# AITRICS/Medical_Tri_Modal_Pilot

Measured on AMD Instinct MI355X. Metric: tri-modal training samples/s (fwd+bwd+AdamW step, per-GPU batch 64), higher is better.
Workload: dtype bf16; 1 GPU; BASELINE configs[1]: vslt_img_txt tri_mbt_vsltcls, 6 layers, d_model 256, batch 64/GPU, TIE-len 1000 (N_v=1005), 224x224 CXR, 128-tok text, dropout 0.1, mbt-only-vslt 1, imgtxt-time 1; global_batch=64, parallelism=dp1

## Files before the change

### include/mtmp.h

```cpp
#ifndef MTMP_H
#define MTMP_H
#include <stdint.h>
#ifdef __cplusplus
extern "C" {
#endif

#define MTMP_F32 0
#define MTMP_BF16 1

int mtmp_abi_version(void);
const char* mtmp_last_error(void);

int mtmp_attn_fwd(int dtype, const void* q, const void* k, const void* v, void* o, const void* res, void* o_res,
                  float* lse, const int32_t* kv_len, const float* key_norms, int B, int N, int H, int ld_qkv, int ld_o,
                  float scale, void* stream);
int mtmp_attn_fwd_grouped(int dtype, int n, const void* const* q, const void* const* k, const void* const* v, void* const* o,
                          const void* const* res, void* const* o_res, float* const* lse, const int32_t* const* kv_len,
                          const int32_t* const* row_start, const float* const* key_norms, const int* N, const int* ld_qkv,
                          const int* ld_o, int B, int H, float scale, void* stream);
int mtmp_attn_bwd_grouped(int dtype, int n, const void* const* q, const void* const* k, const void* const* v,
                          const void* const* o, const void* const* d_o, const float* const* lse, const int32_t* const* kv_len,
                          const int32_t* const* row_start, void* const* dq, void* const* dk, void* const* dv,
                          float* const* delta_ws, const int* N, const int* ld_qkv, const int* ld_o, const int* ld_do,
                          const int* ld_dqkv, int B, int H, float scale, void* stream);
int mtmp_attn_cls_fwd(int dtype, const void* q, const void* k, const void* v, int ld_qkv, const void* res, int ld_res, void* o_cls,
                      void* r1_cls, float* lse, const int32_t* kv_len, const int32_t* row_start, int B, int N, int H, int cls_tok,
                      float scale, void* stream);
int mtmp_attn_cls_bwd(int dtype, const void* q, const void* k, const void* v, int ld_qkv, const void* o_cls, const void* d_o,
                      const float* lse, const int32_t* kv_len, const int32_t* row_start, void* dq, void* dk, void* dv, int ld_dqkv,
                      int B, int N, int H, int cls_tok, float scale, void* stream);
long long mtmp_key_norms_floats(long long rows, int H);
int mtmp_key_norms(int dtype, const void* k, float* out, long long rows, int H, int ld, void* stream);

int mtmp_attn_bwd(int dtype, const void* q, const void* k, const void* v, const void* o, const void* d_o,
                  const float* lse, const int32_t* kv_len, void* dq, void* dk, void* dv, float* delta_ws, int B,
                  int N, int H, int ld_qkv, int ld_o, int ld_do, int ld_dqkv, float scale, void* stream);

int mtmp_ln_gemm(int dtype, const void* x, const float* gamma, const float* beta, const void* w, const float* bias,
                 void* y, void* xn, float* stats, int M, int N, int ldx, int ldy, float eps, int relu, float drop_p,
                 unsigned seed, const unsigned* seed_dev, void* stream);

int mtmp_ln_gemm_qkv(int dtype, const void* x, const float* gamma, const float* beta, const void* w, const float* bias,
                     void* y, void* xn, float* stats, float* key_norms, int M, int ldx, float eps, void* stream);

int mtmp_gemm_nt(int dtype, const void* a, const void* w, const float* bias, const void* res, void* y, int M, int N,
                 int K, int lda, int ldy, int ldr, int act, float drop_p, unsigned seed, const unsigned* seed_dev,
                 const void* gate, float gate_scale, const float* row_scale, int rows_per_scale, void* stream);

long long mtmp_sign_bits_bytes(int M, int N);
int mtmp_ln_gemm_signs(int dtype, const void* x, const float* gamma, const float* beta, const void* w, const float* bias,
                       void* y, void* xn, float* stats, int M, int N, int ldx, int ldy, float eps, float drop_p,
                       unsigned seed, const unsigned* seed_dev, void* signs, void* stream);
int mtmp_gemm_nt_signs(int dtype, const void* a, const void* w, void* y, int M, int N, int lda, int ldy,
                       const void* signs, float gate_scale, void* stream);
int mtmp_gemm_nt_signs_drop(int dtype, const void* a, const void* w, void* y, int M, int N, int lda, int ldy,
                            const void* signs, float gate_scale, float drop_p, unsigned seed, const unsigned* seed_dev,
                            void* a_out, void* stream);

long long mtmp_gemm_tn_ws_floats(int M, int N, int K);
int mtmp_gemm_tn(int dtype, const void* dy, const void* x, float* dw, float* db, float* ws, int M, int N, int K,
                 int ldy, int ldx, void* stream);
int mtmp_gemm_tn_live(int dtype, const void* dy, const void* x, float* dw, float* db, float* ws, int M, int N, int K,
                      int ldy, int ldx, const int32_t* rows_live, void* stream);

int mtmp_dropout_bwd(int dtype, const void* g_in, void* g_out, long long n, unsigned seed, const unsigned* seed_dev,
                     float p, void* stream);

int mtmp_ln_bwd_ws_floats(int M);
int mtmp_ln_bwd(int dtype, const void* z, int ldz, const float* stats, const float* gamma, const void* dy,
                const void* d_res, int ldr, void* dz, float* dgamma_dbeta, float* ws, int M, float eps, void* stream);

int mtmp_gemm_lnbwd_ws_floats(int M);
int mtmp_gemm_lnbwd(int dtype, const void* dy, const void* wt, const void* z, int ldz, const float* stats,
                    const float* gamma, const void* d_res, int ldr, void* dz, float* dgamma_dbeta, float* ws, int M,
                    int K, int ldy, float eps, void* stream);

int mtmp_tie_embed_fwd(int dtype, const float* events, const float* params, const float* ftab, void* out, int n,
                       void* stream);
int mtmp_tie_bwd_ws_floats(int n);
int mtmp_tie_embed_bwd(int dtype, const float* events, const float* params, const void* d_out, float* grads,
                       float* ws, int n, void* stream);

int mtmp_time_embed_fwd(int dtype, const float* events, const float* params, const float* ftab, void* out, int n,
// ... 163 lines not shown
```

### medical_tri_modal_pilot_amd/_lib.py

```python
import ctypes
import os
from ctypes import c_char_p, c_float, c_int, c_longlong, c_uint, c_void_p

_HERE = os.path.dirname(os.path.abspath(__file__))
LIB_PATH = os.environ.get("MTMP_LIB", os.path.join(_HERE, "libmtmp_hip.so"))

F32, BF16 = 0, 1

SIGNATURES = {
    "mtmp_abi_version": (c_int, []),
    "mtmp_last_error": (c_char_p, []),
    "mtmp_attn_fwd": (c_int, [c_int] + [c_void_p] * 9 + [c_int] * 5 + [c_float, c_void_p]),
    "mtmp_attn_cls_fwd": (c_int, [c_int] + [c_void_p] * 3 + [c_int, c_void_p, c_int] + [c_void_p] * 5 + [c_int] * 4 + [c_float, c_void_p]),
    "mtmp_attn_cls_bwd": (c_int, [c_int] + [c_void_p] * 3 + [c_int] + [c_void_p] * 8 + [c_int] * 5 + [c_float, c_void_p]),
    "mtmp_attn_fwd_grouped": (c_int, [c_int, c_int] + [c_void_p] * 13 + [c_int, c_int, c_float, c_void_p]),
    "mtmp_attn_bwd_grouped": (c_int, [c_int, c_int] + [c_void_p] * 17 + [c_int, c_int, c_float, c_void_p]),
    "mtmp_key_norms_floats": (c_longlong, [c_longlong, c_int]),
    "mtmp_key_norms": (c_int, [c_int, c_void_p, c_void_p, c_longlong, c_int, c_int, c_void_p]),
    "mtmp_attn_bwd": (c_int, [c_int] + [c_void_p] * 11 + [c_int] * 7 + [c_float, c_void_p]),
    "mtmp_ln_gemm": (c_int, [c_int] + [c_void_p] * 8 + [c_int] * 4 + [c_float, c_int, c_float, c_uint, c_void_p, c_void_p]),
    "mtmp_ln_gemm_qkv": (c_int, [c_int] + [c_void_p] * 9 + [c_int, c_int, c_float, c_void_p]),
    "mtmp_gemm_nt": (c_int, [c_int] + [c_void_p] * 5 + [c_int] * 7 + [c_float, c_uint, c_void_p, c_void_p, c_float, c_void_p, c_int,
                             c_void_p]),
    "mtmp_gemm_nt_live": (c_int, [c_int] + [c_void_p] * 5 + [c_int] * 7 + [c_float, c_uint, c_void_p, c_void_p, c_float, c_void_p, c_int,
                             c_void_p, c_void_p]),
    "mtmp_sign_bits_bytes": (c_longlong, [c_int, c_int]),
    "mtmp_ln_gemm_signs": (c_int, [c_int] + [c_void_p] * 8 + [c_int] * 4 + [c_float, c_float, c_uint, c_void_p, c_void_p, c_void_p]),
    "mtmp_gemm_nt_signs": (c_int, [c_int] + [c_void_p] * 3 + [c_int] * 4 + [c_void_p, c_float, c_void_p]),
    "mtmp_gemm_nt_signs_drop": (c_int, [c_int] + [c_void_p] * 3 + [c_int] * 4 + [c_void_p, c_float, c_float, c_uint, c_void_p,
                                                                                   c_void_p, c_void_p]),
    "mtmp_ln_gemm_qkv_grouped": (c_int, [c_int, c_int] + [c_void_p] * 11 + [c_float, c_void_p, c_void_p]),
    "mtmp_ln_gemm_signs_grouped": (c_int, [c_int, c_int] + [c_void_p] * 10 + [c_int, c_void_p, c_float, c_float, c_void_p, c_void_p,
                                                                                   c_void_p, c_void_p]),
    "mtmp_gemm_nt_grouped": (c_int, [c_int, c_int] + [c_void_p] * 6 + [c_int, c_int] + [c_void_p] * 3 + [c_int, c_float, c_void_p,
                                                                                                       c_void_p, c_void_p, c_void_p]),
    "mtmp_gemm_nt_signs_drop_grouped": (c_int, [c_int, c_int] + [c_void_p] * 4 + [c_int, c_void_p, c_void_p, c_float, c_float,
                                                                                  c_void_p, c_void_p, c_void_p, c_void_p, c_void_p]),
    "mtmp_gemm_lnbwd_grouped": (c_int, [c_int, c_int] + [c_void_p] * 11 + [c_int, c_void_p, c_float, c_void_p, c_void_p]),
    "mtmp_gemm_tn_group_plan": (c_int, [c_int, c_void_p, c_int, c_int, c_void_p]),
    "mtmp_gemm_tn_grouped": (c_int, [c_int, c_int] + [c_void_p] * 4 + [c_int, c_int] + [c_void_p] * 4 + [c_void_p]),
    "mtmp_gemm_tn_slab_rows": (c_int, [c_int] * 4),
    "mtmp_gemm_lnbwd_slab_rows": (c_int, [c_int]),
    "mtmp_reduce_batch": (c_int, [c_void_p] * 6 + [c_int, c_void_p]),
    "mtmp_reduce_scatter": (c_int, [c_void_p] * 5 + [c_int, c_void_p]),
    "mtmp_stream_input_slab_rows": (c_int, [c_int]),
    "mtmp_stream_input_bwd_partials": (c_int, [c_int] + [c_void_p] * 7 + [c_int] * 3 + [c_float, c_uint, c_void_p, c_void_p, c_void_p, c_void_p]),
    "mtmp_stream_input_bwd_grouped": (c_int, [c_int, c_int] + [c_void_p] * 18),
    "mtmp_stream_input_fwd_add": (c_int, [c_int] + [c_void_p] * 8 + [c_int] * 3 + [c_float, c_float, c_uint, c_void_p, c_void_p, c_void_p, c_void_p, c_int, c_void_p]),
    "mtmp_token_sums": (c_int, [c_int, c_int] + [c_void_p] * 5),
    "mtmp_tie_bwd_slab_rows": (c_int, [c_int]),
    "mtmp_tie_time_embed_bwd_partials": (c_int, [c_int, c_void_p, c_int, c_void_p, c_int, c_int] + [c_void_p] * 6),
    "mtmp_publish_scalar": (c_int, [c_void_p, c_void_p, c_void_p]),
    "mtmp_copy_batch": (c_int, [c_void_p] * 4 + [c_int, c_void_p]),
    "mtmp_stream_lengths": (c_int, [c_void_p] * 4 + [c_int] * 3 + [c_void_p]),
    "mtmp_row_starts": (c_int, [c_void_p, c_void_p, c_int, c_int, c_void_p]),
    "mtmp_image_slots": (c_int, [c_void_p, c_int, c_void_p, c_int, c_int, c_void_p]),
    "mtmp_transpose_batch": (c_int, [c_int, c_void_p, c_void_p, c_void_p, c_void_p, c_int, c_void_p]),
    "mtmp_layernorm_rows": (c_int, [c_int] + [c_void_p] * 4 + [c_longlong, c_int, c_float, c_int, c_int, c_int, c_void_p]),
    "mtmp_layernorm_rows_live": (c_int, [c_int] + [c_void_p] * 4 + [c_longlong, c_int, c_float, c_int, c_int, c_int, c_void_p, c_void_p]),
    "mtmp_swin_window_attn": (c_int, [c_int] + [c_void_p] * 3 + [c_int] * 6 + [c_float, c_void_p]),
    "mtmp_swin_window_attn_live": (c_int, [c_int] + [c_void_p] * 3 + [c_int] * 6 + [c_float, c_void_p, c_void_p]),
    "mtmp_layernorm_rows_bwd_slab_rows": (c_int, [c_longlong, c_int]),
    "mtmp_layernorm_rows_bwd": (c_int, [c_int] + [c_void_p] * 5 + [c_longlong, c_int, c_float, c_void_p]),
    "mtmp_gelu_fwd": (c_int, [c_int, c_void_p, c_void_p, c_longlong, c_void_p]),
    "mtmp_gelu_bwd": (c_int, [c_int, c_void_p, c_void_p, c_void_p, c_longlong, c_void_p]),
    "mtmp_swin_window_attn_bwd": (c_int, [c_int] + [c_void_p] * 5 + [c_int] * 6 + [c_float, c_void_p]),
    "mtmp_swin_window_attn_pad": (c_int, [c_int] + [c_void_p] * 4 + [c_int] * 6 + [c_float, c_void_p, c_void_p]),
# ... 67 lines not shown
```

### medical_tri_modal_pilot_amd/ops.py

```python
import contextlib
import ctypes
from typing import Optional

import torch

from . import _lib, tuning
from ._lib import BF16, F32, call

LN_EPS = 1e-6
N_HEAD, D_MODEL, D_HEAD = 4, 256, 64


def _dt(t: torch.Tensor) -> int:
    if t.dtype == torch.float32:
        return F32
    if t.dtype == torch.bfloat16:
        return BF16
    raise TypeError(f"libmtmp_hip kernels take float32 or bfloat16, got {t.dtype}")


def _p(t: Optional[torch.Tensor], byte_offset: int = 0):
    return None if t is None else ctypes.c_void_p(t.data_ptr() + byte_offset)


# ... 1208 lines not shown
        dqkv = attn_bwd(qkv, o, dr1.view(B, N, D), lse, kv_len).view(M, 3 * D)
    else:
        dqkv = attn_bwd_grouped([qkv], [o], [_packed_full(dr1, B, N)], [lse], [kv_len], [pack])[0].view(M, 3 * D)[:live]
    dwqkv, dbqkv = gemm_tn(dqkv, xn1, out=(sink.wqkv, sink.bqkv) if direct else None, defer=red)
    dz, dg1, db1 = gemm_lnbwd(dqkv, wqkvt, z.view(M, D)[:live], st1, g1, d_res2d=dr1, gb_out=sink.gb1 if direct else None, defer=red)
    if late is not None and red:
        late.append((red, sink if direct else None))
    else:
        if red:
            reduce_batch(red)
        if direct:
            sink.flat.mark_ready(sink.idx)
    dz = dz.view(B, N, D) if pack is None else _packed_full(dz, B, N)
    if direct:
        return dz, None
    grads = (dg1, db1, dwqkv[:D], dbqkv[:D], dwqkv[D:2 * D], dbqkv[D:2 * D], dwqkv[2 * D:], dbqkv[2 * D:],
             dg2, db2, dw1, dc1, dw2, dc2)
    return dz, grads


def attn_cls_fwd(qkv, z, kv_len, pack, cls_tok):
    _gpu(qkv, z)
    B, N, _ = qkv.shape
    es = qkv.element_size()
    o = torch.empty(B, D_MODEL, dtype=qkv.dtype, device=qkv.device)
    r1 = torch.empty_like(o)
    lse = torch.empty(B, N_HEAD, dtype=torch.float32, device=qkv.device)
    call("mtmp_attn_cls_fwd", _dt(qkv), _p(qkv), _p(qkv, D_MODEL * es), _p(qkv, 2 * D_MODEL * es), qkv.stride(1), _p(z), z.stride(1),
         _p(o), _p(r1), _p(lse), _p(kv_len), _p(pack), B, N, N_HEAD, int(cls_tok), D_HEAD ** -0.5, _stream())
    return o, r1, lse


def attn_cls_bwd(qkv, o_cls, d_o, lse, kv_len, pack, cls_tok):
    _gpu(qkv, o_cls, d_o)
    B, N, _ = qkv.shape
    es = qkv.element_size()
    dqkv = torch.empty_like(qkv)
    call("mtmp_attn_cls_bwd", _dt(qkv), _p(qkv), _p(qkv, D_MODEL * es), _p(qkv, 2 * D_MODEL * es), qkv.stride(1), _p(o_cls), _p(_c(d_o)),
         _p(lse), _p(kv_len), _p(pack), _p(dqkv), _p(dqkv, D_MODEL * es), _p(dqkv, 2 * D_MODEL * es), dqkv.stride(1), B, N, N_HEAD,
         int(cls_tok), D_HEAD ** -0.5, _stream())
    return dqkv


_cls_rows_cache = {}


def _cls_rows(B, N, cls_tok, dev):
    key = (B, N, cls_tok, dev.type, dev.index)
    if key not in _cls_rows_cache:
        _cls_rows_cache[key] = (torch.arange(B, dtype=torch.int64) * N + cls_tok).to(dev)
    return _cls_rows_cache[key]


def cls_layer_forward(z, kv_len, P, fused, drop_p, seeds, pack, cls_tok):
    B, N, D = z.shape
    g1, b1, g2, b2, c1, c2 = P[0], P[1], P[8], P[9], P[11], P[13]
    wqkv, bqkv, w1c, w2c, w2t, wqkvt, w1t = fused
    z2 = z.view(B * N, D)
    if pack is not None:
        qkv, xn1, st1 = (t[0] for t in ln_gemm_qkv_grouped([z2], [g1], [b1], [wqkv], [bqkv], [pack])[:3])
    else:
        qkv, xn1, st1 = ln_gemm(z2, g1, b1, wqkv, bqkv, 3 * D)
    qkv = qkv.view(B, N, 3 * D)
    o_cls, r1, lse = attn_cls_fwd(qkv, z, kv_len, pack, cls_tok)
    h, xn2, st2, hsign = ln_gemm(r1, g2, b2, w1c, c1, 4 * D, relu=True, drop_p=drop_p, seed=seeds[0], want_signs=True)
    out = gemm_nt(h, w2c, c2, res2d=r1, drop_p=drop_p, seed=seeds[1])
    rows = pack[:B] if pack is not None else _cls_rows(B, N, cls_tok, z.device)
    return out, (z, kv_len, g1, g2, wqkvt, w1t, w2t, xn1, st1, qkv, o_cls, lse, r1, xn2, st2, h, drop_p, seeds, hsign, pack, rows, cls_tok)


def cls_layer_backward(saved, d_cls, sink=None, late=None):
    z, kv_len, g1, g2, wqkvt, w1t, w2t, xn1, st1, qkv, o_cls, lse, r1, xn2, st2, h, p, seeds, hsign, pack, rows, cls_tok = saved
    B, N, D = z.shape
    M = B * N
    d_out = _c(d_cls).to(z.dtype)
    direct = sink is not None and sink.usable()
    red = [] if tuning.DEFER_REDUCTIONS else None
    if hsign is not None and p > 0 and tuning.FOLD_DROPOUT_BWD:
        dh, dy2 = gemm_nt_signs(d_out, w2t, hsign, 1.0 / (1.0 - p), drop_p=p, seed=seeds[1])
    else:
        dy2 = dropout_bwd(d_out, seeds[1], p) if p > 0 else d_out
        dh = gemm_nt_signs(dy2, w2t, hsign, 1.0 / (1.0 - p)) if hsign is not None else gemm_nt(dy2, w2t, gate=h, gate_scale=1.0 / (1.0 - p))
    dw2, dc2 = gemm_tn(dy2, h, out=(sink.w2, sink.c2) if direct else None, defer=red)
    dw1, dc1 = gemm_tn(dh, xn2, out=(sink.w1, sink.c1) if direct else None, defer=red)
    dr1, dg2, db2 = gemm_lnbwd(dh, w1t, r1, st2, g2, d_res2d=d_out, gb_out=sink.gb2 if direct else None, defer=red)
    dqkv = attn_cls_bwd(qkv, o_cls, dr1, lse, kv_len, pack, cls_tok).view(M, 3 * D)
    z2 = z.view(M, D)
    if pack is not None:
        dwqkv, dbqkv = gemm_tn_grouped([dqkv], [xn1], [(sink.wqkv, sink.bqkv) if direct else None], [red], [pack])[0]
        dz, dg1, db1 = gemm_lnbwd_grouped([dqkv], [wqkvt], [z2], [st1], [g1], [None], [sink.gb1 if direct else None], [red], [pack])[0]
    else:
        dwqkv, dbqkv = gemm_tn(dqkv, xn1, out=(sink.wqkv, sink.bqkv) if direct else None, defer=red)
        dz, dg1, db1 = gemm_lnbwd(dqkv, wqkvt, z2, st1, g1, d_res2d=None, gb_out=sink.gb1 if direct else None, defer=red)
    (dz[cls_tok:] if pack is not None else dz).index_add_(0, rows, dr1)
    if late is not None and red:
        late.append((red, sink if direct else None))
    else:
        if red:
            reduce_batch(red)
        if direct:
            sink.flat.mark_ready(sink.idx)
    if direct:
        return dz.view(B, N, D), None
    grads = (dg1, db1, dwqkv[:D], dbqkv[:D], dwqkv[D:2 * D], dbqkv[D:2 * D], dwqkv[2 * D:], dbqkv[2 * D:],
             dg2, db2, dw1, dc1, dw2, dc2)
    return dz.view(B, N, D), grads




def grouped_ok(z) -> bool:
    return tuning.GROUPED_LAUNCHES and z.dtype == torch.bfloat16


def layer_forward_grouped(zs, kv_lens, Ps, fuseds, drop_p, seeds, packs=None, ffn_rows=None):
    n = len(zs)
    B, D = zs[0].shape[0], D_MODEL
    Ns = [z.shape[1] for z in zs]
    packs = [None] * n if packs is None else list(packs)
    z2 = [z.view(B * N, D) for z, N in zip(zs, Ns)]
    qkv, xn1, st1, knorm = ln_gemm_qkv_grouped(z2, [P[0] for P in Ps], [P[1] for P in Ps], [f[0] for f in fuseds], [f[1] for f in fuseds],
                                               packs)
    qkv = [q.view(B, N, 3 * D) for q, N in zip(qkv, Ns)]
    o, r1, lse = attn_fwd_grouped(qkv, kv_lens, list(zs), knorm, packs)
# ... 363 lines not shown
```

Measured before the change: 8385 samples/s.

## Collapse CLS-only attention layer algebraically to avoid full QKV projection over all tokens

Adds a dedicated CLS-layer path. Only the CLS query is needed, so the query is folded through the key weights and LN gamma/beta, and scores come directly from layer-normed tokens. The value projection is applied once to the attention-weighted normalized input rather than to every row. This removes the full per-token LN+QKV GEMM and the materialized qkv tensor in both forward and backward, replacing them with chunked streaming kernels that do online softmax and partial reductions. It adds several small per-sample kernels and fp32 workspace, and changes accumulation order relative to the GEMM path.

```diff
diff --git a/include/mtmp.h b/include/mtmp.h
--- a/include/mtmp.h
+++ b/include/mtmp.h
@@ -29,6 +29,14 @@
 int mtmp_attn_cls_bwd(int dtype, const void* q, const void* k, const void* v, int ld_qkv, const void* o_cls, const void* d_o,
                       const float* lse, const int32_t* kv_len, const int32_t* row_start, void* dq, void* dk, void* dv, int ld_dqkv,
                       int B, int N, int H, int cls_tok, float scale, void* stream);
+int mtmp_cls_layer_chunk(void);
+long long mtmp_cls_layer_ws_floats(long long B, long long N);
+int mtmp_cls_layer_fwd(int dtype, const void* z, int ldz, const float* gamma, const float* beta, const void* wqkv,
+                       const void* wqkvt, const float* bqkv, const int32_t* kv_len, const int32_t* row_start, int B, int N,
+                       int cls_tok, float eps, float scale, float* ws, void* r1, void* stream);
+int mtmp_cls_layer_bwd(int dtype, const void* z, int ldz, const float* gamma, const float* beta, const void* wqkv,
+                       const void* wqkvt, const int32_t* kv_len, const int32_t* row_start, int B, int N, int cls_tok, float eps,
+                       float scale, float* ws, const void* d_o, void* dz, float* dwqkv, float* dbqkv, float* dgb, void* stream);
 long long mtmp_key_norms_floats(long long rows, int H);
 int mtmp_key_norms(int dtype, const void* k, float* out, long long rows, int H, int ld, void* stream);
 
diff --git a/medical_tri_modal_pilot_amd/_lib.py b/medical_tri_modal_pilot_amd/_lib.py
--- a/medical_tri_modal_pilot_amd/_lib.py
+++ b/medical_tri_modal_pilot_amd/_lib.py
@@ -13,6 +13,10 @@
     "mtmp_attn_fwd": (c_int, [c_int] + [c_void_p] * 9 + [c_int] * 5 + [c_float, c_void_p]),
     "mtmp_attn_cls_fwd": (c_int, [c_int] + [c_void_p] * 3 + [c_int, c_void_p, c_int] + [c_void_p] * 5 + [c_int] * 4 + [c_float, c_void_p]),
     "mtmp_attn_cls_bwd": (c_int, [c_int] + [c_void_p] * 3 + [c_int] + [c_void_p] * 8 + [c_int] * 5 + [c_float, c_void_p]),
+    "mtmp_cls_layer_chunk": (c_int, []),
+    "mtmp_cls_layer_ws_floats": (c_longlong, [c_longlong, c_longlong]),
+    "mtmp_cls_layer_fwd": (c_int, [c_int, c_void_p, c_int] + [c_void_p] * 7 + [c_int] * 3 + [c_float, c_float] + [c_void_p] * 3),
+    "mtmp_cls_layer_bwd": (c_int, [c_int, c_void_p, c_int] + [c_void_p] * 6 + [c_int] * 3 + [c_float, c_float] + [c_void_p] * 7),
     "mtmp_attn_fwd_grouped": (c_int, [c_int, c_int] + [c_void_p] * 13 + [c_int, c_int, c_float, c_void_p]),
     "mtmp_attn_bwd_grouped": (c_int, [c_int, c_int] + [c_void_p] * 17 + [c_int, c_int, c_float, c_void_p]),
     "mtmp_key_norms_floats": (c_longlong, [c_longlong, c_int]),
diff --git a/medical_tri_modal_pilot_amd/csrc/cls_layer.hip b/medical_tri_modal_pilot_amd/csrc/cls_layer.hip
--- /dev/null
+++ b/medical_tri_modal_pilot_amd/csrc/cls_layer.hip
@@ -0,0 +1,562 @@
+#include "common.hip.h"
+
+namespace {
+
+constexpr int D = 256, H = 4, DHD = 64;
+constexpr int CHUNK = 64;
+constexpr int GPB = 8;
+constexpr float LOG2E = 1.4426950408889634f;
+constexpr float NEG = -1e30f;
+
+template <typename T> struct ClsArgs {
+    const T* z; int ldz;
+    const float* gamma; const float* beta;
+    const T* wqkv; const T* wqkvt; const float* bqkv;
+    const int* kv_len; const int* row_start;
+    int B, N, cls_tok, nch;
+    float eps, scale;
+    float *xc, *q, *qt, *qg, *sc0, *P, *mvec, *lse, *stats, *scores, *part, *pml, *dm, *dmg, *dd, *dqt, *dq, *gb;
+    T* r1;
+    const T* d_o;
+    T* dz;
+    float *dwqkv, *dbqkv, *dgb;
+};
+
+struct Geo { bool none, uniform; int kvl, nrows; size_t row0; };
+template <typename T> MTMP_DEV Geo geo(const ClsArgs<T>& p, int b) {
+    Geo g;
+    const int kv_raw = p.kv_len ? p.kv_len[b] : p.N;
+    g.none = p.row_start && kv_raw <= p.cls_tok;
+    g.uniform = !g.none && kv_raw <= 0;
+    g.kvl = g.uniform ? p.N : min(kv_raw, p.N);
+    g.nrows = p.row_start ? max(min(kv_raw, p.N), 0) : p.N;
+    g.row0 = p.row_start ? (size_t)p.row_start[b] : (size_t)b * p.N;
+    return g;
+}
+
+template <typename T> MTMP_DEV void ld8(const T* ptr, float (&o)[8]) {
+    const Frag<T> f = frag_load<T>(ptr);
+#pragma unroll
+    for (int j = 0; j < 8; ++j) o[j] = to_f32(f.v[j]);
+}
+template <typename T> MTMP_DEV void st8(T* ptr, const float (&v)[8]) {
+    Frag<T> f;
+#pragma unroll
+    for (int j = 0; j < 8; ++j) f.v[j] = from_f32<T>(v[j]);
+    frag_store<T>(ptr, f);
+}
+MTMP_DEV void ld8w(const float* ptr, float (&o)[8]) {
+    const f32x4 a = ld4f(ptr), b = ld4f(ptr + 4);
+    o[0] = a[0]; o[1] = a[1]; o[2] = a[2]; o[3] = a[3]; o[4] = b[0]; o[5] = b[1]; o[6] = b[2]; o[7] = b[3];
+}
+MTMP_DEV float grp_sum(float v) {
+    v += dpp_row<0x128>(v);
+    v += dpp_row<0x124>(v);
+    v += dpp_row<0x122>(v);
+    v += dpp_row<0x121>(v);
+    const auto r = __builtin_amdgcn_permlane16_swap(__float_as_uint(v), __float_as_uint(v), false, false);
+    return __uint_as_float(r[0]) + __uint_as_float(r[1]);
+}
+MTMP_DEV float block_sum(float v, float* red) {
+    v = wave_sum(v);
+    __syncthreads();
+    if ((threadIdx.x & 63) == 0) red[threadIdx.x >> 6] = v;
+    __syncthreads();
+    return (red[0] + red[1]) + (red[2] + red[3]);
+}
+
+template <typename T> __global__ __launch_bounds__(256) void cls_prepare_kernel(ClsArgs<T> p) {
+    __shared__ float sx[D], sq[D], red[4];
+    const int b = blockIdx.x, t = threadIdx.x;
+    const Geo g = geo(p, b);
+    if (g.none) {
+        p.xc[b * D + t] = 0.f;
+        p.q[b * D + t] = 0.f;
+        for (int h = 0; h < H; ++h) { p.qt[(b * H + h) * D + t] = 0.f; p.qg[(b * H + h) * D + t] = 0.f; }
+        if (t < H) p.sc0[b * H + t] = 0.f;
+        return;
+    }
+    const float zc = to_f32(p.z[(g.row0 + p.cls_tok) * p.ldz + t]);
+    const float mean = block_sum(zc, red) * (1.0f / D);
+    const float d = zc - mean;
+    const float sigma = sqrtf(block_sum(d * d, red) * (1.0f / (D - 1)));
+    const float rs = 1.0f / (sigma + p.eps);
+    const float gm = p.gamma[t], be = p.beta[t];
+    const float x = fmaf(gm, d * rs, be);
+    sx[t] = x;
+    p.xc[b * D + t] = x;
+    __syncthreads();
+    float a = p.bqkv[t];
+#pragma unroll 8
+    for (int k = 0; k < D; ++k) a = fmaf(to_f32(p.wqkvt[(size_t)k * 3 * D + t]), sx[k], a);
+    sq[t] = a;
+    p.q[b * D + t] = a;
+    __syncthreads();
+    const float c2 = p.scale * LOG2E;
+    for (int h = 0; h < H; ++h) {
+        float w = 0.f;
+#pragma unroll 8
+        for (int dd = 0; dd < DHD; ++dd) w = fmaf(to_f32(p.wqkv[(size_t)(D + DHD * h + dd) * D + t]), sq[DHD * h + dd], w);
+        if (g.uniform) w = 0.f;
+        p.qt[(b * H + h) * D + t] = w;
+        p.qg[(b * H + h) * D + t] = w * c2 * gm;
+        const float c = block_sum(w * c2 * be, red);
+        if (t == 0) p.sc0[b * H + h] = c;
+    }
+}
+
+template <typename T> __global__ __launch_bounds__(256) void cls_fwd_pass_kernel(ClsArgs<T> p) {
+    __shared__ __attribute__((aligned(16))) float sred[GPB * D];
+    __shared__ float sm[GPB][H], sl[GPB][H];
+    const int b = blockIdx.y, ch = blockIdx.x, tid = threadIdx.x;
+    const Geo g = geo(p, b);
+    const int r0 = ch * CHUNK;
+    if (g.none || r0 >= g.kvl) return;
+    const int r1 = min(r0 + CHUNK, g.kvl);
+    const int gi = tid >> 5, ll = tid & 31, c0 = 8 * ll;
+    float qg[H][8], sc0[H], m[H], l[H], acc[H][8];
+#pragma unroll
+    for (int h = 0; h < H; ++h) {
+        ld8w(p.qg + (size_t)(b * H + h) * D + c0, qg[h]);
+        sc0[h] = p.sc0[b * H + h];
+        m[h] = NEG;
+        l[h] = 0.f;
+#pragma unroll
+        for (int i = 0; i < 8; ++i) acc[h][i] = 0.f;
+    }
+    const T* zb = p.z + g.row0 * p.ldz + c0;
+    Frag<T> nxt = frag_load<T>(zb + (size_t)min(r0 + gi, r1 - 1) * p.ldz);
+#pragma unroll 2
+    for (int it = 0; it < CHUNK / GPB; ++it) {
+        const int r = r0 + gi + GPB * it;
+        const bool live = r < r1;
+        const size_t rc = (size_t)min(r, r1 - 1);
+        const Frag<T> cur = nxt;
+        nxt = frag_load<T>(zb + (size_t)min(r + GPB, r1 - 1) * p.ldz);
+        float v[8];
+#pragma unroll
+        for (int i = 0; i < 8; ++i) v[i] = to_f32(cur.v[i]);
+        float s = 0.f;
+#pragma unroll
+        for (int i = 0; i < 8; ++i) s += v[i];
+        const float mean = grp_sum(s) * (1.0f / D);
+        float s2 = 0.f;
+#pragma unroll
+        for (int i = 0; i < 8; ++i) { v[i] -= mean; s2 = fmaf(v[i], v[i], s2); }
+        const float sigma = sqrtf(grp_sum(s2) * (1.0f / (D - 1)));
+        const float rs = 1.0f / (sigma + p.eps);
+        float sc[H];
+#pragma unroll
+        for (int i = 0; i < 8; ++i) v[i] *= rs;
+#pragma unroll
+        for (int h = 0; h < H; ++h) {
+            float a = 0.f;
+#pragma unroll
+            for (int i = 0; i < 8; ++i) a = fmaf(qg[h][i], v[i], a);
+            sc[h] = grp_sum(a) + sc0[h];
+        }
+        if (live && ll == 0) {
+            const size_t gr = g.row0 + rc;
+            *reinterpret_cast<f32x2*>(p.stats + 2 * gr) = f32x2{mean, rs};
+            *reinterpret_cast<f32x4*>(p.scores + 4 * gr) = f32x4{sc[0], sc[1], sc[2], sc[3]};
+        }
+#pragma unroll
+        for (int h = 0; h < H; ++h) {
+            const float se = live ? sc[h] : NEG;
+            const float mn = fmaxf(m[h], se);
+            const float a = fast_exp2(m[h] - mn);
+            const float e = live ? fast_exp2(sc[h] - mn) : 0.f;
+            l[h] = fmaf(l[h], a, e);
+#pragma unroll
+            for (int i = 0; i < 8; ++i) acc[h][i] = fmaf(acc[h][i], a, e * v[i]);
+            m[h] = mn;
+        }
+    }
+    if (ll == 0) {
+#pragma unroll
+        for (int h = 0; h < H; ++h) { sm[gi][h] = m[h]; sl[gi][h] = l[h]; }
+    }
+    __syncthreads();
+    const size_t pb = (size_t)(b * p.nch + ch) * H;
+#pragma unroll
+    for (int h = 0; h < H; ++h) {
+        float M = sm[0][h];
+#pragma unroll
+        for (int k = 1; k < GPB; ++k) M = fmaxf(M, sm[k][h]);
+        const float f = fast_exp2(m[h] - M);
+        float t8[8];
+#pragma unroll
+        for (int i = 0; i < 8; ++i) t8[i] = acc[h][i] * f;
+        *reinterpret_cast<f32x4*>(sred + gi * D + c0) = f32x4{t8[0], t8[1], t8[2], t8[3]};
+        *reinterpret_cast<f32x4*>(sred + gi * D + c0 + 4) = f32x4{t8[4], t8[5], t8[6], t8[7]};
+        __syncthreads();
+        float a = 0.f;
+#pragma unroll
+        for (int k = 0; k < GPB; ++k) a += sred[k * D + tid];
+        p.part[(pb + h) * D + tid] = a;
+        if (tid == 0) {
+            float L = 0.f;
+#pragma unroll
+            for (int k = 0; k < GPB; ++k) L = fmaf(sl[k][h], fast_exp2(sm[k][h] - M), L);
+            p.pml[(pb + h) * 2] = M;
+            p.pml[(pb + h) * 2 + 1] = L;
+        }
+        __syncthreads();
+    }
+}
+
+template <typename T> __global__ __launch_bounds__(256) void cls_combine_kernel(ClsArgs<T> p) {
+    __shared__ float smv[H][D];
+    const int b = blockIdx.x, t = threadIdx.x;
+    const Geo g = geo(p, b);
+    if (g.none) {
+        p.r1[b * D + t] = from_f32<T>(0.f);
+        for (int h = 0; h < H; ++h) { p.P[(b * H + h) * D + t] = 0.f; p.mvec[(b * H + h) * D + t] = 0.f; }
+        if (t < H) p.lse[b * H + t] = 0.f;
+        return;
+    }
+    const int nl = (g.kvl + CHUNK - 1) / CHUNK;
+    const float gm = p.gamma[t], be = p.beta[t];
+    for (int h = 0; h < H; ++h) {
+        const float* ml = p.pml + ((size_t)b * p.nch * H + h) * 2;
+        float M = NEG;
+        for (int c = 0; c < nl; ++c) M = fmaxf(M, ml[(size_t)c * H * 2]);
+        float L = 0.f, a = 0.f;
+        for (int c = 0; c < nl; ++c) {
+            const float f = fast_exp2(ml[(size_t)c * H * 2] - M);
+            L = fmaf(ml[(size_t)c * H * 2 + 1], f, L);
+            a = fmaf(p.part[((size_t)(b * p.nch + c) * H + h) * D + t], f, a);
+        }
+        const float Ph = a / L;
+        const float mv = fmaf(gm, Ph, be);
+        p.P[(b * H + h) * D + t] = Ph;
+        p.mvec[(b * H + h) * D + t] = mv;
+        smv[h][t] = mv;
+        if (t == 0) p.lse[b * H + h] = M + log2f(L);
+    }
+    __syncthreads();
+    const int hh = t >> 6;
+    float o = p.bqkv[2 * D + t];
+#pragma unroll 8
+    for (int k = 0; k < D; ++k) o = fmaf(to_f32(p.wqkvt[(size_t)k * 3 * D + 2 * D + t]), smv[hh][k], o);
+    p.r1[b * D + t] = from_f32<T>(o + to_f32(p.z[(g.row0 + p.cls_tok) * p.ldz + t]));
+}
+
+template <typename T> __global__ __launch_bounds__(256) void cls_bwd_prologue_kernel(ClsArgs<T> p) {
+    __shared__ float sdo[D], red[4];
+    const int b = blockIdx.x, t = threadIdx.x;
+    const Geo g = geo(p, b);
+    if (g.none) {
+        for (int h = 0; h < H; ++h) { p.dm[(b * H + h) * D + t] = 0.f; p.dmg[(b * H + h) * D + t] = 0.f; }
+        if (t < H) p.dd[b * H + t] = 0.f;
+        return;
+    }
+    sdo[t] = to_f32(p.d_o[b * D + t]);
+    __syncthreads();
+    const float gm = p.gamma[t];
+    for (int h = 0; h < H; ++h) {
+        float a = 0.f;
+#pragma unroll 8
+        for (int dd = 0; dd < DHD; ++dd) a = fmaf(to_f32(p.wqkv[(size_t)(2 * D + DHD * h + dd) * D + t]), sdo[DHD * h + dd], a);
+        p.dm[(b * H + h) * D + t] = a;
+        p.dmg[(b * H + h) * D + t] = a * gm;
+        const float s = block_sum(a * gm * p.P[(b * H + h) * D + t], red);
+        if (t == 0) p.dd[b * H + h] = -s;
+    }
+}
+
+template <typename T> __global__ __launch_bounds__(256) void cls_bwd_pass_kernel(ClsArgs<T> p) {
+    __shared__ __attribute__((aligned(16))) float sred[GPB * D];
+    __shared__ float ss[GPB][H];
+    const int b = blockIdx.y, ch = blockIdx.x, tid = threadIdx.x;
+    const Geo g = geo(p, b);
+    const int r0 = ch * CHUNK;
+    if (r0 >= g.nrows) return;
+    const int rend = min(r0 + CHUNK, g.nrows);
+    const int gi = tid >> 5, ll = tid & 31, c0 = 8 * ll;
+    T* dzb = p.dz + g.row0 * D + c0;
+    if (g.none || r0 >= g.kvl) {
+        const float zero[8] = {0.f, 0.f, 0.f, 0.f, 0.f, 0.f, 0.f, 0.f};
+        for (int r = r0 + gi; r < rend; r += GPB) st8<T>(dzb + (size_t)r * D, zero);
+        return;
+    }
+    const int r1 = min(r0 + CHUNK, g.kvl);
+    float dmg[H][8], qn[H][8], dd[H], lse[H], A[H][8], S[H];
+    const float qs = g.uniform ? 0.f : 1.0f / LOG2E;
+#pragma unroll
+    for (int h = 0; h < H; ++h) {
+        ld8w(p.dmg + (size_t)(b * H + h) * D + c0, dmg[h]);
+        ld8w(p.qg + (size_t)(b * H + h) * D + c0, qn[h]);
+        dd[h] = p.dd[b * H + h];
+        lse[h] = p.lse[b * H + h];
+        S[h] = 0.f;
+#pragma unroll
+        for (int i = 0; i < 8; ++i) { qn[h][i] *= qs; A[h][i] = 0.f; }
+    }
+    const T* zb = p.z + g.row0 * p.ldz + c0;
+    const float* stb = p.stats + 2 * g.row0;
+    const float* scb = p.scores + 4 * g.row0;
+    size_t rn = (size_t)min(r0 + gi, r1 - 1);
+    Frag<T> nxt = frag_load<T>(zb + rn * p.ldz);
+    f32x2 nst = *reinterpret_cast<const f32x2*>(stb + 2 * rn);
+    f32x4 nsc = *reinterpret_cast<const f32x4*>(scb + 4 * rn);
+#pragma unroll 2
+    for (int it = 0; it < CHUNK / GPB; ++it) {
+        const int r = r0 + gi + GPB * it;
+        const bool live = r < r1;
+        const Frag<T> cur = nxt;
+        const f32x2 st = nst;
+        const f32x4 sc = nsc;
+        rn = (size_t)min(r + GPB, r1 - 1);
+        nxt = frag_load<T>(zb + rn * p.ldz);
+        nst = *reinterpret_cast<const f32x2*>(stb + 2 * rn);
+        nsc = *reinterpret_cast<const f32x4*>(scb + 4 * rn);
+        float v[8];
+#pragma unroll
+        for (int i = 0; i < 8; ++i) v[i] = to_f32(cur.v[i]);
+        const float mean = st[0], rs = st[1];
+#pragma unroll
+        for (int i = 0; i < 8; ++i) v[i] = (v[i] - mean) * rs;
+        float pr[H], ds[H];
+#pragma unroll
+        for (int h = 0; h < H; ++h) {
+            float a = 0.f;
+#pragma unroll
+            for (int i = 0; i < 8; ++i) a = fmaf(dmg[h][i], v[i], a);
+            pr[h] = fast_exp2(sc[h] - lse[h]);
+            const float dpx = grp_sum(a) + dd[h];
+            ds[h] = g.uniform ? 0.f : pr[h] * dpx;
+        }
+        float gg[8], sg = 0.f, sgx = 0.f;
+#pragma unroll
+        for (int i = 0; i < 8; ++i) {
+            float a = 0.f;
+#pragma unroll
+            for (int h = 0; h < H; ++h) a = fmaf(pr[h], dmg[h][i], fmaf(ds[h], qn[h][i], a));
+            gg[i] = a;
+            sg += a;
+            sgx = fmaf(a, v[i], sgx);
+        }
+        sg = grp_sum(sg);
+        sgx = grp_sum(sgx);
+        const float sigma = 1.0f / rs - p.eps;
+        const float mg = sg * (1.0f / D), kx = sgx / ((float)(D - 1) * sigma);
+        float out[8];
+#pragma unroll
+        for (int i = 0; i < 8; ++i) out[i] = live ? (gg[i] - mg) * rs - v[i] * kx : 0.f;
+        if (r < rend) st8<T>(dzb + (size_t)r * D, out);
+#pragma unroll
+        for (int h = 0; h < H; ++h) {
+            const float dsl = live ? ds[h] : 0.f;
+            S[h] += dsl;
+#pragma unroll
+            for (int i = 0; i < 8; ++i) A[h][i] = fmaf(dsl, v[i], A[h][i]);
+        }
+    }
+    if (ll == 0) {
+#pragma unroll
+        for (int h = 0; h < H; ++h) ss[gi][h] = S[h];
+    }
+    const size_t pb = (size_t)(b * p.nch + ch) * H;
+#pragma unroll
+    for (int h = 0; h < H; ++h) {
+        *reinterpret_cast<f32x4*>(sred + gi * D + c0) = f32x4{A[h][0], A[h][1], A[h][2], A[h][3]};
+        *reinterpret_cast<f32x4*>(sred + gi * D + c0 + 4) = f32x4{A[h][4], A[h][5], A[h][6], A[h][7]};
+        __syncthreads();
+        float a = 0.f;
+#pragma unroll
+        for (int k = 0; k < GPB; ++k) a += sred[k * D + tid];
+        p.part[(pb + h) * D + tid] = a;
+        if (tid == 0) {
+            float s = 0.f;
+#pragma unroll
+            for (int k = 0; k < GPB; ++k) s += ss[k][h];
+            p.pml[(pb + h) * 2] = s;
+        }
+        __syncthreads();
+    }
+}
+
+template <typename T> __global__ __launch_bounds__(256) void cls_bwd_sample_kernel(ClsArgs<T> p) {
+    __shared__ float sdqt[H][D], sdq[D], red[4];
+    const int b = blockIdx.x, t = threadIdx.x;
+    const Geo g = geo(p, b);
+    if (g.none) {
+        for (int h = 0; h < H; ++h) p.dqt[(b * H + h) * D + t] = 0.f;
+        p.dq[b * D + t] = 0.f;
+        p.gb[b * 2 * D + t] = 0.f;
+        p.gb[b * 2 * D + D + t] = 0.f;
+        return;
+    }
+    const int nl = (g.kvl + CHUNK - 1) / CHUNK;
+    const float gm = p.gamma[t], be = p.beta[t];
+    float gbg = 0.f, gbb = 0.f;
+    for (int h = 0; h < H; ++h) {
+        float A = 0.f, S = 0.f;
+        for (int c = 0; c < nl; ++c) {
+            A += p.part[((size_t)(b * p.nch + c) * H + h) * D + t];
+            S += p.pml[((size_t)(b * p.nch + c) * H + h) * 2];
+        }
+        const float dqt = p.scale * fmaf(gm, A, be * S);
+        p.dqt[(b * H + h) * D + t] = dqt;
+        sdqt[h][t] = dqt;
+        const float dm = p.dm[(b * H + h) * D + t], sq = p.scale * p.qt[(b * H + h) * D + t];
+        gbg += fmaf(dm, p.P[(b * H + h) * D + t], sq * A);
+        gbb += fmaf(sq, S, dm);
+    }
+    __syncthreads();
+    const int hh = t >> 6;
+    float a = 0.f;
+#pragma unroll 8
+    for (int k = 0; k < D; ++k) a = fmaf(to_f32(p.wqkvt[(size_t)k * 3 * D + D + t]), sdqt[hh][k], a);
+    p.dq[b * D + t] = a;
+    sdq[t] = a;
+    __syncthreads();
+    float ex = 0.f;
+#pragma unroll 8
+    for (int n = 0; n < D; ++n) ex = fmaf(to_f32(p.wqkv[(size_t)n * D + t]), sdq[n], ex);
+    const size_t crow = g.row0 + p.cls_tok;
+    const float zc = to_f32(p.z[crow * p.ldz + t]);
+    const float mean = block_sum(zc, red) * (1.0f / D);
+    const float d = zc - mean;
+    const float sigma = sqrtf(block_sum(d * d, red) * (1.0f / (D - 1)));
+    const float rs = 1.0f / (sigma + p.eps);
+    const float xh = d * rs;
+    const bool key = p.cls_tok < g.kvl;
+    float gg = ex * gm;
+    for (int h = 0; h < H; ++h) {
+        const float dmg = p.dmg[(b * H + h) * D + t];
+        const float dpx = block_sum(dmg * xh, red) + p.dd[b * H + h];
+        const float pr = key ? fast_exp2(p.scores[4 * crow + h] - p.lse[b * H + h]) : 0.f;
+        const float ds = g.uniform ? 0.f : pr * dpx;
+        gg += fmaf(pr, dmg, ds * p.scale * p.qt[(b * H + h) * D + t] * gm);
+    }
+    const float sg = block_sum(gg, red), sgx = block_sum(gg * xh, red);
+    const float mg = sg * (1.0f / D), kx = sgx / ((float)(D - 1) * sigma);
+    p.dz[crow * D + t] = from_f32<T>((gg - mg) * rs - xh * kx + to_f32(p.d_o[b * D + t]));
+    p.gb[b * 2 * D + t] = fmaf(ex, xh, gbg);
+    p.gb[b * 2 * D + D + t] = gbb + ex;
+}
+
+constexpr int WROWS = 8;
+template <typename T> __global__ __launch_bounds__(256) void cls_bwd_params_kernel(ClsArgs<T> p) {
+    const int blk = blockIdx.x, t = threadIdx.x;
+    if (blk >= 3 * D / WROWS) {
+        const int which = blk - 3 * D / WROWS;
+        float a = 0.f;
+        for (int b = 0; b < p.B; ++b) a += p.gb[(size_t)b * 2 * D + which * D + t];
+        p.dgb[which * D + t] = a;
+        return;
+    }
+    const int n0 = blk * WROWS, type = n0 / D, nn = n0 % D, h = nn / DHD;
+    float acc[WROWS], bias = 0.f;
+#pragma unroll
+    for (int j = 0; j < WROWS; ++j) acc[j] = 0.f;
+    for (int b = 0; b < p.B; ++b) {
+        const bool none = p.row_start && p.kv_len[b] <= p.cls_tok;
+        const float v = type == 0 ? p.xc[b * D + t] : type == 1 ? p.dqt[(b * H + h) * D + t] : p.mvec[(b * H + h) * D + t];
+        float a[WROWS];
+#pragma unroll
+        for (int j = 0; j < WROWS; ++j)
+            a[j] = type == 0 ? p.dq[b * D + nn + j] : type == 1 ? p.q[b * D + nn + j] : (none ? 0.f : to_f32(p.d_o[b * D + nn + j]));
+#pragma unroll
+        for (int j = 0; j < WROWS; ++j) acc[j] = fmaf(a[j], v, acc[j]);
+        if (t < WROWS) bias += type == 0 ? p.dq[b * D + nn + t] : type == 1 ? 0.f : (none ? 0.f : to_f32(p.d_o[b * D + nn + t]));
+    }
+#pragma unroll
+    for (int j = 0; j < WROWS; ++j) p.dwqkv[(size_t)(n0 + j) * D + t] = acc[j];
+    if (t < WROWS) p.dbqkv[n0 + t] = bias;
+}
+
+struct WsLayout { size_t xc, q, qt, qg, sc0, P, mvec, lse, stats, scores, part, pml, dm, dmg, dd, dqt, dq, gb, total; };
+WsLayout ws_layout(long long B, long long N) {
+    WsLayout w;
+    size_t o = 0;
+    auto take = [&](size_t n) { const size_t r = o; o += (n + 3) & ~(size_t)3; return r; };
+    const size_t nch = (size_t)(N + CHUNK - 1) / CHUNK, b = (size_t)B, rows = b * (size_t)N;
+    w.xc = take(b * D); w.q = take(b * D); w.qt = take(b * H * D); w.qg = take(b * H * D); w.sc0 = take(b * H);
+    w.P = take(b * H * D); w.mvec = take(b * H * D); w.lse = take(b * H);
+    w.stats = take(rows * 2); w.scores = take(rows * 4);
+    w.part = take(b * nch * H * D); w.pml = take(b * nch * H * 2);
+    w.dm = take(b * H * D); w.dmg = take(b * H * D); w.dd = take(b * H);
+    w.dqt = take(b * H * D); w.dq = take(b * D); w.gb = take(b * 2 * D);
+    w.total = o;
+    return w;
+}
+
+template <typename T>
+ClsArgs<T> make_args(const void* z, int ldz, const float* gamma, const float* beta, const void* wqkv, const void* wqkvt,
+                     const float* bqkv, const int32_t* kv_len, const int32_t* row_start, int B, int N, int cls_tok, float eps,
+                     float scale, float* ws) {
+    const WsLayout w = ws_layout(B, N);
+    ClsArgs<T> a{};
+    a.z = (const T*)z; a.ldz = ldz; a.gamma = gamma; a.beta = beta;
+    a.wqkv = (const T*)wqkv; a.wqkvt = (const T*)wqkvt; a.bqkv = bqkv;
+    a.kv_len = kv_len; a.row_start = row_start;
+    a.B = B; a.N = N; a.cls_tok = cls_tok; a.nch = (N + CHUNK - 1) / CHUNK; a.eps = eps; a.scale = scale;
+    a.xc = ws + w.xc; a.q = ws + w.q; a.qt = ws + w.qt; a.qg = ws + w.qg; a.sc0 = ws + w.sc0; a.P = ws + w.P; a.mvec = ws + w.mvec;
+    a.lse = ws + w.lse; a.stats = ws + w.stats; a.scores = ws + w.scores; a.part = ws + w.part; a.pml = ws + w.pml;
+    a.dm = ws + w.dm; a.dmg = ws + w.dmg; a.dd = ws + w.dd; a.dqt = ws + w.dqt; a.dq = ws + w.dq; a.gb = ws + w.gb;
+    return a;
+}
+
+bool cls_layer_ok(int B, int N, int cls_tok, int ldz) {
+    return B > 0 && N > 0 && (long long)B * N < (1ll << 28) && cls_tok >= 0 && cls_tok < N && ldz >= D && ldz % 8 == 0;
+}
+
+template <typename T> void launch_fwd(ClsArgs<T> a, hipStream_t st) {
+    hipLaunchKernelGGL(cls_prepare_kernel<T>, dim3(a.B), dim3(256), 0, st, a);
+    hipLaunchKernelGGL(cls_fwd_pass_kernel<T>, dim3(a.nch, a.B), dim3(256), 0, st, a);
+    hipLaunchKernelGGL(cls_combine_kernel<T>, dim3(a.B), dim3(256), 0, st, a);
+}
+template <typename T> void launch_bwd(ClsArgs<T> a, hipStream_t st) {
+    hipLaunchKernelGGL(cls_bwd_prologue_kernel<T>, dim3(a.B), dim3(256), 0, st, a);
+    hipLaunchKernelGGL(cls_bwd_pass_kernel<T>, dim3(a.nch, a.B), dim3(256), 0, st, a);
+    hipLaunchKernelGGL(cls_bwd_sample_kernel<T>, dim3(a.B), dim3(256), 0, st, a);
+    hipLaunchKernelGGL(cls_bwd_params_kernel<T>, dim3(3 * D / WROWS + 2), dim3(256), 0, st, a);
+}
+}
+
+extern "C" int mtmp_cls_layer_chunk(void) { return CHUNK; }
+extern "C" long long mtmp_cls_layer_ws_floats(long long B, long long N) { return B > 0 && N > 0 ? (long long)ws_layout(B, N).total : 0; }
+
+extern "C" int mtmp_cls_layer_fwd(int dtype, const void* z, int ldz, const float* gamma, const float* beta, const void* wqkv,
+                                  const void* wqkvt, const float* bqkv, const int32_t* kv_len, const int32_t* row_start, int B,
+                                  int N, int cls_tok, float eps, float scale, float* ws, void* r1, void* stream) {
+    MTMP_CHECK_ARG(z && gamma && beta && wqkv && wqkvt && bqkv && ws && r1, "mtmp_cls_layer_fwd: null pointer");
+    MTMP_CHECK_ARG(cls_layer_ok(B, N, cls_tok, ldz) && (!row_start || kv_len),
+                   "mtmp_cls_layer_fwd: bad argument (B=%d N=%d cls=%d ld=%d)", B, N, cls_tok, ldz);
+    hipStream_t st = (hipStream_t)stream;
+    if (dtype == 0) {
+        ClsArgs<float> a = make_args<float>(z, ldz, gamma, beta, wqkv, wqkvt, bqkv, kv_len, row_start, B, N, cls_tok, eps, scale, ws);
+        a.r1 = (float*)r1;
+        launch_fwd<float>(a, st);
+    } else if (dtype == 1) {
+        ClsArgs<bf16> a = make_args<bf16>(z, ldz, gamma, beta, wqkv, wqkvt, bqkv, kv_len, row_start, B, N, cls_tok, eps, scale, ws);
+        a.r1 = (bf16*)r1;
+        launch_fwd<bf16>(a, st);
+    } else { mtmp_set_error("mtmp_cls_layer_fwd: unknown dtype %d", dtype); return MTMP_ERR_ARG; }
+    MTMP_CHECK_LAUNCH("mtmp_cls_layer_fwd");
+    return MTMP_OK;
+}
+
+extern "C" int mtmp_cls_layer_bwd(int dtype, const void* z, int ldz, const float* gamma, const float* beta, const void* wqkv,
+                                  const void* wqkvt, const int32_t* kv_len, const int32_t* row_start, int B, int N, int cls_tok,
+                                  float eps, float scale, float* ws, const void* d_o, void* dz, float* dwqkv, float* dbqkv,
+                                  float* dgb, void* stream) {
+    MTMP_CHECK_ARG(z && gamma && beta && wqkv && wqkvt && ws && d_o && dz && dwqkv && dbqkv && dgb, "mtmp_cls_layer_bwd: null pointer");
+    MTMP_CHECK_ARG(cls_layer_ok(B, N, cls_tok, ldz) && (!row_start || kv_len),
+                   "mtmp_cls_layer_bwd: bad argument (B=%d N=%d cls=%d ld=%d)", B, N, cls_tok, ldz);
+    hipStream_t st = (hipStream_t)stream;
+    if (dtype == 0) {
+        ClsArgs<float> a = make_args<float>(z, ldz, gamma, beta, wqkv, wqkvt, nullptr, kv_len, row_start, B, N, cls_tok, eps, scale, ws);
+        a.d_o = (const float*)d_o; a.dz = (float*)dz; a.dwqkv = dwqkv; a.dbqkv = dbqkv; a.dgb = dgb;
+        launch_bwd<float>(a, st);
+    } else if (dtype == 1) {
+        ClsArgs<bf16> a = make_args<bf16>(z, ldz, gamma, beta, wqkv, wqkvt, nullptr, kv_len, row_start, B, N, cls_tok, eps, scale, ws);
+        a.d_o = (const bf16*)d_o; a.dz = (bf16*)dz; a.dwqkv = dwqkv; a.dbqkv = dbqkv; a.dgb = dgb;
+        launch_bwd<bf16>(a, st);
+    } else { mtmp_set_error("mtmp_cls_layer_bwd: unknown dtype %d", dtype); return MTMP_ERR_ARG; }
+    MTMP_CHECK_LAUNCH("mtmp_cls_layer_bwd");
+    return MTMP_OK;
+}
diff --git a/medical_tri_modal_pilot_amd/ops.py b/medical_tri_modal_pilot_amd/ops.py
--- a/medical_tri_modal_pilot_amd/ops.py
+++ b/medical_tri_modal_pilot_amd/ops.py
@@ -1284,7 +1284,70 @@
     return _cls_rows_cache[key]
 
 
+def cls_layer_ok(z) -> bool:
+    return z.dim() == 3 and z.shape[2] == D_MODEL and z.is_contiguous()
+
+
 def cls_layer_forward(z, kv_len, P, fused, drop_p, seeds, pack, cls_tok):
+    if not cls_layer_ok(z):
+        return cls_layer_forward_kv(z, kv_len, P, fused, drop_p, seeds, pack, cls_tok)
+    _gpu(z)
+    B, N, D = z.shape
+    g1, b1, g2, b2, c1, c2 = P[0], P[1], P[8], P[9], P[11], P[13]
+    wqkv, bqkv, w1c, w2c, w2t, wqkvt, w1t = fused
+    ws = torch.empty(_lib.lib().mtmp_cls_layer_ws_floats(B, N), dtype=torch.float32, device=z.device)
+    r1 = torch.empty(B, D, dtype=z.dtype, device=z.device)
+    call("mtmp_cls_layer_fwd", _dt(z), _p(z), z.stride(1), _p(g1), _p(b1), _p(wqkv), _p(wqkvt), _p(bqkv), _p(kv_len), _p(pack),
+         B, N, int(cls_tok), LN_EPS, D_HEAD ** -0.5, _p(ws), _p(r1), _stream())
+    h, xn2, st2, hsign = ln_gemm(r1, g2, b2, w1c, c1, 4 * D, relu=True, drop_p=drop_p, seed=seeds[0], want_signs=True)
+    out = gemm_nt(h, w2c, c2, res2d=r1, drop_p=drop_p, seed=seeds[1])
+    return out, (_CLS_COLLAPSED, z, kv_len, g1, b1, g2, wqkv, wqkvt, w1t, w2t, ws, r1, xn2, st2, h, drop_p, seeds, hsign, pack, cls_tok)
+
+
+_CLS_COLLAPSED = "cls_layer"
+
+
+def cls_layer_backward(saved, d_cls, sink=None, late=None):
+    if saved[0] is not _CLS_COLLAPSED:
+        return cls_layer_backward_kv(saved, d_cls, sink, late)
+    _, z, kv_len, g1, b1, g2, wqkv, wqkvt, w1t, w2t, ws, r1, xn2, st2, h, p, seeds, hsign, pack, cls_tok = saved
+    B, N, D = z.shape
+    d_out = _c(d_cls).to(z.dtype)
+    direct = sink is not None and sink.usable()
+    red = [] if tuning.DEFER_REDUCTIONS else None
+    if hsign is not None and p > 0 and tuning.FOLD_DROPOUT_BWD:
+        dh, dy2 = gemm_nt_signs(d_out, w2t, hsign, 1.0 / (1.0 - p), drop_p=p, seed=seeds[1])
+    else:
+        dy2 = dropout_bwd(d_out, seeds[1], p) if p > 0 else d_out
+        dh = gemm_nt_signs(dy2, w2t, hsign, 1.0 / (1.0 - p)) if hsign is not None else gemm_nt(dy2, w2t, gate=h, gate_scale=1.0 / (1.0 - p))
+    dw2, dc2 = gemm_tn(dy2, h, out=(sink.w2, sink.c2) if direct else None, defer=red)
+    dw1, dc1 = gemm_tn(dh, xn2, out=(sink.w1, sink.c1) if direct else None, defer=red)
+    dr1, dg2, db2 = gemm_lnbwd(dh, w1t, r1, st2, g2, d_res2d=d_out, gb_out=sink.gb2 if direct else None, defer=red)
+    dev = z.device
+    dz = torch.empty(B * N, D, dtype=z.dtype, device=dev)
+    if direct:
+        dwqkv, dbqkv, gb1 = sink.wqkv, sink.bqkv, sink.gb1
+    else:
+        dwqkv = torch.empty(3 * D, D, dtype=torch.float32, device=dev)
+        dbqkv = torch.empty(3 * D, dtype=torch.float32, device=dev)
+        gb1 = torch.empty(2 * D, dtype=torch.float32, device=dev)
+    call("mtmp_cls_layer_bwd", _dt(z), _p(z), z.stride(1), _p(g1), _p(b1), _p(wqkv), _p(wqkvt), _p(kv_len), _p(pack), B, N,
+         int(cls_tok), LN_EPS, D_HEAD ** -0.5, _p(ws), _p(_c(dr1)), _p(dz), _p(dwqkv), _p(dbqkv), _p(gb1), _stream())
+    if late is not None and red:
+        late.append((red, sink if direct else None))
+    else:
+        if red:
+            reduce_batch(red)
+        if direct:
+            sink.flat.mark_ready(sink.idx)
+    if direct:
+        return dz.view(B, N, D), None
+    grads = (gb1[:D], gb1[D:], dwqkv[:D], dbqkv[:D], dwqkv[D:2 * D], dbqkv[D:2 * D], dwqkv[2 * D:], dbqkv[2 * D:],
+             dg2, db2, dw1, dc1, dw2, dc2)
+    return dz.view(B, N, D), grads
+
+
+def cls_layer_forward_kv(z, kv_len, P, fused, drop_p, seeds, pack, cls_tok):
     B, N, D = z.shape
     g1, b1, g2, b2, c1, c2 = P[0], P[1], P[8], P[9], P[11], P[13]
     wqkv, bqkv, w1c, w2c, w2t, wqkvt, w1t = fused
@@ -1301,7 +1364,7 @@
     return out, (z, kv_len, g1, g2, wqkvt, w1t, w2t, xn1, st1, qkv, o_cls, lse, r1, xn2, st2, h, drop_p, seeds, hsign, pack, rows, cls_tok)
 
 
-def cls_layer_backward(saved, d_cls, sink=None, late=None):
+def cls_layer_backward_kv(saved, d_cls, sink=None, late=None):
     z, kv_len, g1, g2, wqkvt, w1t, w2t, xn1, st1, qkv, o_cls, lse, r1, xn2, st2, h, p, seeds, hsign, pack, rows, cls_tok = saved
     B, N, D = z.shape
     M = B * N
```

Result: no change. 8340 samples/s (-0.5%).
